# TUI-NICR/EMSANet

Hardware: AMD Instinct MI355X
Metric: images/sec (640x480 RGB-D, bs=32/GPU) fwd+bwd (higher is better)
Workload: dtype f32; 1 GPU; BASELINE.json configs[1]: full EMSANet RGB-D (resnet34-NBt1D x2, SE-add fusion, PPM, semantic+instance+orientation+scene heads), 640x480, bs=32/GPU, f32, train mode (BN batch stats, Dropout2d), step = fwd + bwd (fixed output cotangents) + grad all-reduce + SGD-nesterov update at lr 0 (fixed weights) replayed from a hipGraph; global_batch=32, parallelism=dp1, weights=random init (deterministic), mode=train-hipgraph

## Files before the change

### emsanet_amd/_lib.py

```python
import ctypes
import os
from ctypes import POINTER, Structure, c_char_p, c_float, c_int, c_int8, c_int32, c_int64, c_uint32, c_void_p

LIB_PATH = os.environ.get('EMSA_LIB') or os.path.join(
    os.path.dirname(os.path.abspath(__file__)), 'lib', 'libemsanet_hip.so')


class EmsaPackJob(Structure):
    _fields_ = [('src', c_void_p), ('dst0', c_void_p), ('dst1', c_void_p), ('cout', c_int32),
                ('cin', c_int32), ('kh', c_int32), ('kw', c_int32), ('kind', c_int32),
                ('first_block', c_int32), ('cout_total', c_int32), ('cout_off', c_int32),
                ('cin_total', c_int32), ('cin_off', c_int32)]


class EmsaDropoutJob(Structure):
    _fields_ = [('offset', c_int64), ('c', c_int32), ('layer_id', c_uint32), ('p', c_float),
                ('pad_', c_int32)]


class EmsaConvGeom(Structure):
    _fields_ = [
        ('n_img', c_int32),
        ('in_h', c_int32), ('in_w', c_int32),
        ('out_h', c_int32), ('out_w', c_int32),
# ... 41 lines not shown
    'emsa_conv_relu_bits_words': (c_int64, [c_int64, c_int32]),
    'emsa_conv1d_wino_bnb': (c_int, [_GP, _P, _P, _P, _P, c_int32, _P, c_int32, _P, _P, _P, _P, _P,
                                     c_int32, _P]),
    'emsa_conv_igemm_bnb_t': (c_int, [c_int32, _GP, _P, _P, _P, _P, c_int32, _P, c_int32, _P, _P, _P, _P,
                                      _P, c_int32, _P]),
    'emsa_bn_bwd_apply_rows_t': (c_int, [c_int32, _P, _P, _P, _P, _P, _P, c_int32, c_int32, c_int64,
                                         c_int32, c_int32, _P, _P, _P, _P]),
    'emsa_conv1d_wino': (c_int, [_GP, _P, _P, _P, _P, _P, _P, _P, _P, c_int32, _P, c_int32, c_int32, _P,
                                 _P, _P]),
    'emsa_memset_async': (c_int, [_P, c_int32, c_int64, _P]),
    'emsa_graph_count_nodes': (c_int, [_P, POINTER(c_int32), POINTER(c_int32), POINTER(c_int32)]),
    'emsa_graph_replace_memsets': (c_int, [_P, POINTER(c_int32)]),
    'emsa_dropout2d_mask_batch': (c_int, [_P, _P, c_int32, c_int32, c_int32, c_uint32, _P, _P]),
    'emsa_to_nhwc_t': (c_int, [c_int32, _P, _P, c_int32, c_int32, c_int32, c_int32, c_int64, c_int64,
                               c_int64, c_int64, _P]),
    'emsa_conv1d_wino_resmask_supported': (c_int, [_GP, c_int32]),
    'emsa_conv1d_wino_resmask': (c_int, [_GP, _P, _P, _P, _P, c_int32, _P, _P]),
    'emsa_bn_act_fwd_wbits': (c_int, [_P, _P, _P, _P, _P, _P, c_int32, c_int64, c_int32, c_int32, _P, _P]),
    'emsa_bn_act_fwd_raff': (c_int, [_P] * 8 + [c_int32, c_int64, c_int32, c_int32, _P, c_int32, _P]),
    'emsa_bn_bwd_reduce_wbits': (c_int, [_P, _P, _P, _P, _P, _P, c_int32, c_int64, c_int32, _P, _P]),
    'emsa_bn_bwd_apply_wbits': (c_int, [_P] * 8 + [c_int32, c_int32, c_int64, c_int32, c_int32] + [_P] * 5),
    'emsa_conv1d_wino_inbn': (c_int, [_GP, _P, _P, _P, _P, _P, _P, _P, c_int32, _P, _P]),
    'emsa_conv_wgrad_inbn': (c_int, [_GP, _P, _P, _P, _P, _P, _P, _P, _P]),
    'emsa_conv_wgrad_inbn_t': (c_int, [c_int32, _GP, _P, _P, _P, _P, _P, _P, _P, _P]),
    'emsa_conv_wgrad_multi_inbn_t': (c_int, [c_int32, c_int32, _GP, POINTER(c_void_p), POINTER(c_void_p),
                                             POINTER(c_void_p), POINTER(c_void_p), _P,
                                             POINTER(c_void_p), POINTER(c_void_p), _P]),
    'emsa_conv1d_rs_inbn_t': (c_int, [c_int32, _GP, _P, _P, _P, _P, _P, _P, _P, c_int32, _P]),
    'emsa_bn_bwd_reduce_aff_t': (c_int, [c_int32, _P, _P, _P, _P, _P, _P, c_int32, c_int64, c_int32, _P, _P]),
    'emsa_bn_bwd_apply_aff_t': (c_int, [c_int32, _P, _P, _P, _P, _P, _P, _P, _P, c_int32, c_int32, c_int64,
# ... 247 lines not shown
```

### emsanet_amd/csrc/conv_mfma.hip

```cpp
#include "common.h"

#include <type_traits>
#include <vector>

#include "prof.h"

namespace {

struct ProfSlotImpl {
  hipEvent_t a, b;
  int cls;
  double flops, bytes;
};
std::vector<ProfSlotImpl> g_prof_pool;
size_t g_prof_used = 0;
int g_prof_every = 0;
int g_prof_seen[kProfClasses] = {0};
double g_prof_next_flops = 0.0;
const char* const kProfNames[kProfClasses] = {
    "conv_igemm_kernel<128,128,2,2>", "conv_igemm_kernel<128,64,4,2>",
    "conv_igemm_kernel<64,64,2,2>",   "conv_igemm_kernel<128,32,4,1>",
    "conv_wgrad_kernel<64,32,7,2,1,2>", "conv_wgrad_kernel<128,128,1,2,2,1> (unused)",
    "conv_wgrad_kernel<64,64,1,2,2,1>", "conv_wgrad_kernel<64,64,3,2,2,1>|conv_wgrad1d_wino_kernel<64,64> (1-D convs)",
    "conv1d_wino_kernel (1-D 3x1/1x3 convs)", "conv_h_kernel (16-bit igemm)",
// ... 956 lines not shown
  const bool dok = co0 + col4 < p.n_ch, xok = ci0 + col4 < p.k_ch;
  const uint32_t dadd = dok ? (uint32_t)(co0 + col4) * ES : 0u, dmask = dok ? 0u : kOOB;
  const uint32_t xadd = xok ? (uint32_t)(ci0 + col4) * ES : 0u, xmask = xok ? 0u : kOOB;

  typename Raw4<T>::type re_raw[2], rx_raw[4];
  float4 bsum = emsa_zero4();
  uint32_t x_real = 0;
  float* const xbnS = smem + NP * 4 * (BCO + BCI);
  if constexpr (XBN) {
    if (tid < 2 * BCI) {
      const int ch = ci0 + (tid & (BCI - 1));
      const float* src = tid < BCI ? p.in_scale : p.in_shift;
      xbnS[tid] = ch < p.k_ch ? src[ch] : 0.f;
    }
  }
  auto load_regs = [&](int s) {
    const int k = s * PK + lane - 1;
    const bool valid = lane < XROWS && k >= 0 && k < p.M;
    const uint32_t ku = valid ? (uint32_t)k : 0u;
    const uint32_t img = fast_div(ku, p.div_al);
    const uint32_t line = fast_div(ku, p.div_l);
    const int b_ = (int)(ku - __umul24(line, (uint32_t)p.L));
    const int a_ = (int)(line - __umul24(img, (uint32_t)p.A));
    const int a2 = a_ + dline;
    const bool in_line = valid && b_ < p.Lr;
    const uint32_t off_d = in_line
        ? (__umul24(img, (uint32_t)p.dy_simg) + __umul24((uint32_t)a_, (uint32_t)p.dy_sa) +
           __umul24((uint32_t)b_, (uint32_t)p.dy_sb)) * ES : kOOB;
    const uint32_t off_x = (in_line && a2 >= 0 && a2 < p.A)
        ? (__umul24(img, (uint32_t)p.in_simg) + __umul24((uint32_t)a2, (uint32_t)p.in_sa) +
           __umul24((uint32_t)b_, (uint32_t)p.in_sb)) * ES : kOOB;
    const uint32_t off_xl = b_ == p.L - 1 ? kOOB : off_x;
    const uint32_t off_xr = b_ == 0 ? kOOB : off_x;
    const int l0 = (2 * pr) * 4;
    const uint32_t o_e0 = (uint32_t)__builtin_amdgcn_ds_bpermute(l0 + 4, (int)off_d);
    const uint32_t o_e1 = (uint32_t)__builtin_amdgcn_ds_bpermute(l0 + 8, (int)off_d);
    const uint32_t o_d0 = (uint32_t)__builtin_amdgcn_ds_bpermute(l0, (int)off_xl);
    const uint32_t o_d1 = (uint32_t)__builtin_amdgcn_ds_bpermute(l0 + 4, (int)off_x);
    const uint32_t o_d2 = (uint32_t)__builtin_amdgcn_ds_bpermute(l0 + 8, (int)off_x);
    const uint32_t o_d3 = (uint32_t)__builtin_amdgcn_ds_bpermute(l0 + 12, (int)off_xr);
    re_raw[0] = buf_ld4raw<T>(rs_dy, (o_e0 + dadd) | dmask);
    re_raw[1] = buf_ld4raw<T>(rs_dy, (o_e1 + dadd) | dmask);
    rx_raw[0] = buf_ld4raw<T>(rs_in, (o_d0 + xadd) | xmask);
    rx_raw[1] = buf_ld4raw<T>(rs_in, (o_d1 + xadd) | xmask);
    rx_raw[2] = buf_ld4raw<T>(rs_in, (o_d2 + xadd) | xmask);
    rx_raw[3] = buf_ld4raw<T>(rs_in, (o_d3 + xadd) | xmask);
    if constexpr (XBN)
      x_real = (~o_d0 >> 31) | ((~o_d1 >> 31) << 1) | ((~o_d2 >> 31) << 2) | ((~o_d3 >> 31) << 3);
  };
  auto add4 = [](const float4& a, const float4& b) {
    return make_float4(a.x + b.x, a.y + b.y, a.z + b.z, a.w + b.w);
  };
  auto sub4 = [](const float4& a, const float4& b) {
    return make_float4(a.x - b.x, a.y - b.y, a.z - b.z, a.w - b.w);
  };
  auto store_lds = [&]() {
    const float4 re[2] = {raw_f4(re_raw[0], (T*)nullptr), raw_f4(re_raw[1], (T*)nullptr)};
    float4 rx[4] = {raw_f4(rx_raw[0], (T*)nullptr), raw_f4(rx_raw[1], (T*)nullptr),
                    raw_f4(rx_raw[2], (T*)nullptr), raw_f4(rx_raw[3], (T*)nullptr)};
    if constexpr (XBN) {
      typedef float f2 __attribute__((ext_vector_type(2)));
// ... 1489 lines not shown
```

### emsanet_amd/csrc/conv_wino.hip

```cpp
#include <cstdlib>

#include "common.h"
#include "prof.h"

namespace {

constexpr int kWK = 16;
constexpr int kWLD = kWK;
constexpr int kPairs = 32;

typedef unsigned int u32x4w __attribute__((ext_vector_type(4)));
typedef __bf16 wbf16x8 __attribute__((ext_vector_type(8)));
constexpr uint32_t kOOBw = 0x80000000u;
__device__ __forceinline__ __amdgpu_buffer_rsrc_t wrsrc(const void* p, uint32_t bytes) {
  return __builtin_amdgcn_make_buffer_rsrc(const_cast<void*>(p), 0, (int)bytes, 0x00020000);
}
__device__ __forceinline__ float4 wbuf_ld4(__amdgpu_buffer_rsrc_t r, uint32_t off) {
  return __builtin_bit_cast(float4, __builtin_amdgcn_raw_buffer_load_b128(r, (int)off, 0, 0));
}
__device__ __forceinline__ float4 wbuf_ld4s(__amdgpu_buffer_rsrc_t r, uint32_t voff, uint32_t soff) {
  return __builtin_bit_cast(float4,
                            __builtin_amdgcn_raw_buffer_load_b128(r, (int)voff, (int)soff, 0));
}
typedef float wf32x2 __attribute__((ext_vector_type(2)));
// ... 31 lines not shown

__device__ __forceinline__ int wswz(int row, int c4) {
  return row * kWLD + (c4 ^ (((row >> 2) & 3) << 2));
}

__device__ __forceinline__ uint32_t wdiv(uint32_t n, uint32_t mul, uint32_t sh) {
  return (__umulhi(n, mul) + n) >> sh;
}

#ifndef EMSA_WINO_ST_AUX
#define EMSA_WINO_ST_AUX 0
#endif
#ifndef EMSA_WINO_PRIO
#define EMSA_WINO_PRIO 2
#endif
template <int kWN, bool BF16 = false, bool BNB = false, bool INBN = false>
__global__ __launch_bounds__(256, kWN == 64 ? (BNB ? 4 : 5) : 6) void conv1d_wino_kernel(const WinoArgs p) {
  constexpr int NT = kWN / 32;
  constexpr int NC4 = kWN / 4;
  constexpr int RG = 256 / NC4;
  constexpr int PXI = 64 / RG;
  constexpr int BLD = 4 * kWN * 4 / 256;
  extern __shared__ __attribute__((aligned(16))) float smem[];
  float* const As = smem;
  float* const Bs = smem + 4 * kPairs * kWLD;
  float* const Ts = Bs + 4 * kWN * kWLD;

  const int tid = threadIdx.x, lane = tid & 63, wave = __builtin_amdgcn_readfirstlane(tid >> 6);
  const int l31 = lane & 31, lh = lane >> 5;
  const int wg = emsa_xcd_remap(blockIdx.x, gridDim.x);
  const int nt = wg % p.tiles_n, mt = wg / p.tiles_n;
  const int q0 = mt * kPairs, n0 = nt * kWN;
// ... 13 lines not shown
      int al = 0;
      if (q < p.MP) {
        const int line = (int)wdiv((uint32_t)q, p.mul_pl, p.sh_pl);
        const int pp = q - line * p.PL;
        const int img = (int)wdiv((uint32_t)line, p.mul_a, p.sh_a);
        const int a = line - img * p.A;
        const int b = 2 * pp - 1 + rr;
        if (b >= 0 && b < p.L)
          off = (uint32_t)(img * p.in_simg + a * p.in_sa + b * p.in_sb + c4) * 4u;
        al = a;
      }
      a_base[j] = off;
      a_line[j] = al;
    }
  };
  setup_a(mt);
#pragma unroll
  for (int j = 0; j < BLD; ++j) {
    const int rowid = (tid >> 2) + 64 * j;
    const int comp = rowid / kWN, n = n0 + (rowid % kWN);
    b_voff[j] = n < p.n_ch ? (uint32_t)((comp * p.n_ch + n) * p.k_ch + c4) * 4u : kOOBw;
  }
  auto set_row = [&](int r) {
    const int dr = p.R == 3 ? r - 1 : 0;
#pragma unroll
    for (int j = 0; j < 2; ++j) {
      const int al = a_line[j] + dr;
      const bool ok = !(a_base[j] & kOOBw) && al >= 0 && al < p.A;
      a_voff[j] = ok ? a_base[j] + (uint32_t)(dr * p.in_sa * 4) : kOOBw;
    }
  };
  const uint32_t last_oob = (p.ksteps_c - 1) * kWK + c4 < p.c_in ? 0u : kOOBw;
  float4 ra[2], rb[BLD];
  auto load_regs = [&](int s) {
    const int r = s >= 2 * p.ksteps_c ? 2 : (s >= p.ksteps_c ? 1 : 0);
    const int ch = (s - r * p.ksteps_c) * kWK;
    if (ch == 0) set_row(r);
    const uint32_t sa = (uint32_t)ch * 4u, sb = (uint32_t)(r * p.c_in + ch) * 4u;
    const uint32_t pm = ch + kWK > p.c_in ? 0xFFFFFFFFu : 0u;
#pragma unroll
    for (int j = 0; j < 2; ++j) ra[j] = wbuf_ld4s(rs_in, a_voff[j] | (last_oob & pm), sa);
#pragma unroll
    for (int j = 0; j < BLD; ++j) rb[j] = wbuf_ld4s(rs_u, b_voff[j] | (last_oob & pm), sb);
  };
  auto store_lds = [&](int s) {
    if constexpr (INBN) {
      const int kt = p.ksteps_c * kWK;
      const float4 sc = emsa_ld4(Ts + s * kWK + c4), sh = emsa_ld4(Ts + kt + s * kWK + c4);
#pragma unroll
// ... 9 lines not shown
                            __builtin_amdgcn_fmed3f(hi.y, 0.f, cap));
      }
    }
#pragma unroll
    for (int j = 0; j < 2; ++j) emsa_st4(As + wswz((tid >> 2) + 64 * j, c4), ra[j]);
#pragma unroll
    for (int j = 0; j < BLD; ++j) emsa_st4(Bs + wswz((tid >> 2) + 64 * j, c4), rb[j]);
  };

  const int ra_ = wave == 0 ? 0 : wave == 2 ? 2 : 1;
  const int rb_ = wave == 2 ? 1 : wave == 3 ? 3 : 2;
  const float sg = wave == 1 ? 1.f : -1.f;

  load_regs(0);
  f32x16 acc[NT];
#pragma unroll
  for (int t = 0; t < NT; ++t)
#pragma unroll
    for (int r = 0; r < 16; ++r) acc[t][r] = 0.f;

  if constexpr (INBN) {
    const int kt = p.ksteps_c * kWK;
    for (int i = tid; i < kt; i += 256) {
      Ts[i] = i < p.c_in ? p.in_scale[i] : 0.f;
      Ts[kt + i] = i < p.c_in ? p.in_shift[i] : 0.f;
    }
    __syncthreads();
  }
  store_lds(0);
  __syncthreads();
  for (int s = 0; s < p.ksteps; ++s) {
    const bool has_next = s + 1 < p.ksteps;
#if EMSA_WINO_PRIO == 2
    __builtin_amdgcn_s_setprio(3);
#endif
    if (has_next) load_regs(s + 1);
    const int sw = ((l31 >> 2) & 3) << 2;
    const float* a0 = As + (ra_ * kPairs + l31) * kWLD;
    const float* a1 = As + (rb_ * kPairs + l31) * kWLD;
    const float* b = Bs + (wave * kWN + l31) * kWLD;
#if EMSA_WINO_PRIO != 0
    __builtin_amdgcn_s_setprio(1);
#endif
    if constexpr (BF16) {
      const int c0 = (lh << 2) ^ sw, c1 = ((lh + 2) << 2) ^ sw;
      const float4 p0 = emsa_ld4(a0 + c0), q0 = emsa_ld4(a1 + c0);
// ... 12 lines not shown
        acc[u] = __builtin_amdgcn_mfma_f32_32x32x16_bf16(va, vb, acc[u], 0, 0, 0);
      }
    } else {
#pragma unroll
    for (int t = 0; t < kWK / 8; ++t) {
      const int co = ((lh + 2 * t) << 2) ^ sw;
      const float4 x0 = emsa_ld4(a0 + co), x1 = emsa_ld4(a1 + co);
      const wf32x2 sg2 = {sg, sg};
      const wf32x2 vlo = __builtin_elementwise_fma(wf32x2{x1.x, x1.y}, sg2, wf32x2{x0.x, x0.y});
      const wf32x2 vhi = __builtin_elementwise_fma(wf32x2{x1.z, x1.w}, sg2, wf32x2{x0.z, x0.w});
      const float4 v = make_float4(vlo.x, vlo.y, vhi.x, vhi.y);
      float4 fb[NT];
#pragma unroll
      for (int u = 0; u < NT; ++u) fb[u] = emsa_ld4(b + u * 32 * kWLD + co);
#pragma unroll
      for (int u = 0; u < NT; ++u)
        acc[u] = __builtin_amdgcn_mfma_f32_32x32x2f32(v.x, fb[u].x, acc[u], 0, 0, 0);
#pragma unroll
      for (int u = 0; u < NT; ++u)
        acc[u] = __builtin_amdgcn_mfma_f32_32x32x2f32(v.y, fb[u].y, acc[u], 0, 0, 0);
#pragma unroll
      for (int u = 0; u < NT; ++u)
        acc[u] = __builtin_amdgcn_mfma_f32_32x32x2f32(v.z, fb[u].z, acc[u], 0, 0, 0);
#pragma unroll
      for (int u = 0; u < NT; ++u)
        acc[u] = __builtin_amdgcn_mfma_f32_32x32x2f32(v.w, fb[u].w, acc[u], 0, 0, 0);
    }
    }
#if EMSA_WINO_PRIO != 0
    __builtin_amdgcn_s_setprio(0);
#endif
    __syncthreads();
    if (has_next) store_lds(s + 1);
    __syncthreads();
  }

  constexpr int SLD = kWN + 4;
  constexpr int HP = kPairs / 2;
  constexpr uint32_t kNoPix = 0xFFFFFFFFu;
  float* const stage = smem;
  const int col4 = tid % NC4, n = n0 + col4 * 4;
  const int rgi = tid / NC4;
  const bool nok = n < p.n_ch;
  uint32_t lane_pix = kNoPix;
  {
    const int q = q0 + (lane >> 1);
    if (q < p.MP) {
      const int line = (int)wdiv((uint32_t)q, p.mul_pl, p.sh_pl);
      const int pp = q - line * p.PL;
      const int img = (int)wdiv((uint32_t)line, p.mul_a, p.sh_a);
      const int a = line - img * p.A;
      const int b = 2 * pp + (lane & 1);
      if (b < p.L) lane_pix = (uint32_t)(img * p.px_simg + a * p.px_sa + b * p.px_sb);
    }
  }
  wf32x2 ylo[PXI], yhi[PXI];
  uint32_t opix[PXI];
  bool ok[PXI];
  const float4 bv = (nok && p.bias) ? emsa_ld4(p.bias + n) : emsa_zero4();
  const wf32x2 blo = {bv.x, bv.y}, bhi = {bv.z, bv.w};
  const float sgo = (rgi & 1) ? -1.f : 1.f;
  const wf32x2 sg2o = {sgo, sgo};
  const int m03row = (rgi & 1) ? 3 : 0;
#pragma unroll
  for (int k = 0; k < PXI; ++k) {
    const uint32_t o = (uint32_t)__builtin_amdgcn_ds_bpermute((rgi + RG * k) * 4, (int)lane_pix);
    ok[k] = nok && o != kNoPix;
    opix[k] = o;
  }
  const __amdgpu_buffer_rsrc_t rs_out = wrsrc(p.out, kOOBw);
  const __amdgpu_buffer_rsrc_t rs_res = wrsrc(p.residual, kOOBw);
  const __amdgpu_buffer_rsrc_t rs_msk = wrsrc(p.mask_src, kOOBw);
  const __amdgpu_buffer_rsrc_t rs_mb = wrsrc(p.mask_bits, kOOBw);
  float4 rres[PXI], rmsk[PXI];
  wu32x2 rbits[PXI];
#pragma unroll
  for (int k = 0; k < PXI; ++k) {
    const bool live = ok[k];
    if (p.residual)
      rres[k] = wbuf_ld4(rs_res, live ? (opix[k] * (uint32_t)p.ld_res + (uint32_t)n) * 4u : kOOBw);
    if (p.mask_src)
      rmsk[k] = wbuf_ld4(rs_msk, live ? (opix[k] * (uint32_t)p.ld_mask + (uint32_t)n) * 4u : kOOBw);
    if constexpr (kWN == 64) {
      if (p.mask_bits)
        rbits[k] = __builtin_bit_cast(
            wu32x2, __builtin_amdgcn_raw_buffer_load_b64(
                        rs_mb, (int)(live ? (opix[k] * (uint32_t)p.tiles_n + (uint32_t)nt) * 8u
                                          : kOOBw), 0, 0));
    }
  }
#pragma unroll
  for (int h = 0; h < 2; ++h) {
  if (h) __syncthreads();
#pragma unroll
  for (int t = 0; t < NT; ++t)
#pragma unroll
    for (int r = 8 * h; r < 8 * h + 8; ++r) {
      const int row = (r & 3) + 8 * (r >> 2) + 4 * lh;
      stage[(wave * HP + row - HP * h) * SLD + t * 32 + l31] = acc[t][r];
    }
  __syncthreads();
#pragma unroll
  for (int k = h * (PXI / 2); k < (h + 1) * (PXI / 2); ++k) {
    const int px = rgi + RG * k;
    const int prl = (px >> 1) - HP * h;
    const float4 m1 = emsa_ld4(stage + (1 * HP + prl) * SLD + col4 * 4);
    const float4 m2 = emsa_ld4(stage + (2 * HP + prl) * SLD + col4 * 4);
    const float4 m03 = emsa_ld4(stage + (m03row * HP + prl) * SLD + col4 * 4);
    const wf32x2 tlo = wf32x2{m2.x, m2.y} + wf32x2{m03.x, m03.y};
    const wf32x2 thi = wf32x2{m2.z, m2.w} + wf32x2{m03.z, m03.w};
    ylo[k] = __builtin_elementwise_fma(tlo, sg2o, wf32x2{m1.x, m1.y}) + blo;
    yhi[k] = __builtin_elementwise_fma(thi, sg2o, wf32x2{m1.z, m1.w}) + bhi;
  }
  }

  if (p.stats != nullptr) {
    __syncthreads();
    float* red = smem;
    float* tmean = smem + RG * kWN;
    int* scnt = reinterpret_cast<int*>(tmean + kWN);
    wf32x2 s1lo = {0.f, 0.f}, s1hi = {0.f, 0.f};
    float wgt[PXI];
    int cnt = 0;
#pragma unroll
    for (int k = 0; k < PXI; ++k) {
      wgt[k] = ok[k] ? 1.f : 0.f;
      const wf32x2 w2 = {wgt[k], wgt[k]};
      s1lo = __builtin_elementwise_fma(ylo[k], w2, s1lo);
      s1hi = __builtin_elementwise_fma(yhi[k], w2, s1hi);
      cnt += ok[k] ? 1 : 0;
    }
// ... 26 lines not shown
    }
    __syncthreads();
    emsa_st4(red + rgi * kWN + col4 * 4, make_float4(s2lo.x, s2lo.y, s2hi.x, s2hi.y));
    __syncthreads();
    if (tid < kWN && n0 + tid < p.n_ch) {
      float a2 = 0.f;
#pragma unroll
      for (int g = 0; g < RG; ++g) a2 += red[g * kWN + tid];
      p.stats[((size_t)1 * p.tiles_m + mt) * p.n_ch + n0 + tid] = a2;
    }
  }

  {
    wf32x2 sclo = {1.f, 1.f}, schi = {1.f, 1.f}, shlo = {0.f, 0.f}, shhi = {0.f, 0.f};
    constexpr bool bnb = BNB;
    const bool affine = p.scale != nullptr && !bnb;
    if (p.scale != nullptr && nok) {
      const float4 sc = emsa_ld4(p.scale + n), sh = emsa_ld4(p.shift + n);
      sclo = wf32x2{sc.x, sc.y}; schi = wf32x2{sc.z, sc.w};
      shlo = wf32x2{sh.x, sh.y}; shhi = wf32x2{sh.z, sh.w};
    }
    wf32x2 mulo = {0.f, 0.f}, muhi = {0.f, 0.f};
    wf32x2 b0lo = {0.f, 0.f}, b0hi = {0.f, 0.f}, b1lo = {0.f, 0.f}, b1hi = {0.f, 0.f};
    if (bnb && nok) {
      const float4 mu = emsa_ld4(p.bnb_mean + n);
      mulo = wf32x2{mu.x, mu.y}; muhi = wf32x2{mu.z, mu.w};
    }
#pragma unroll
    for (int k = 0; k < PXI; ++k) {
      const bool live = ok[k];
      wf32x2 vlo = ylo[k], vhi = yhi[k];
      if (affine) {
        vlo = __builtin_elementwise_fma(vlo, sclo, shlo);
        vhi = __builtin_elementwise_fma(vhi, schi, shhi);
      }
      auto gate = [&](float4& q) {
        const uint32_t t0 = rbits[k].x >> col4, t1 = rbits[k].y >> col4;
        q.x = __uint_as_float(__float_as_uint(q.x) & (uint32_t)__builtin_amdgcn_sbfe((int)t0, 0, 1));
        q.y = __uint_as_float(__float_as_uint(q.y) & (uint32_t)__builtin_amdgcn_sbfe((int)t0, 16, 1));
        q.z = __uint_as_float(__float_as_uint(q.z) & (uint32_t)__builtin_amdgcn_sbfe((int)t1, 0, 1));
        q.w = __uint_as_float(__float_as_uint(q.w) & (uint32_t)__builtin_amdgcn_sbfe((int)t1, 16, 1));
      };
      if (p.residual) {
        float4 rr = rres[k];
        if constexpr (kWN == 64) {
          if (p.mask_res) gate(rr);
        }
        vlo += wf32x2{rr.x, rr.y};
        vhi += wf32x2{rr.z, rr.w};
      }
      float4 v = make_float4(vlo.x, vlo.y, vhi.x, vhi.y);
      if constexpr (bnb) {
        const float4 tt = rmsk[k];
        const wf32x2 alo = __builtin_elementwise_fma(wf32x2{tt.x, tt.y}, sclo, shlo);
        const wf32x2 ahi = __builtin_elementwise_fma(wf32x2{tt.z, tt.w}, schi, shhi);
        const float lv = live ? 1.f : 0.f;
        v.x = alo.x > 0.f ? v.x * lv : 0.f; v.y = alo.y > 0.f ? v.y * lv : 0.f;
        v.z = ahi.x > 0.f ? v.z * lv : 0.f; v.w = ahi.y > 0.f ? v.w * lv : 0.f;
        const wf32x2 glo = {v.x, v.y}, ghi = {v.z, v.w};
        b0lo += glo; b0hi += ghi;
        b1lo = __builtin_elementwise_fma(glo, wf32x2{tt.x, tt.y} - mulo, b1lo);
        b1hi = __builtin_elementwise_fma(ghi, wf32x2{tt.z, tt.w} - muhi, b1hi);
      } else if (p.mask_src) {
        const float4 mm = rmsk[k];
        v.x = mm.x > 0.f ? v.x : 0.f; v.y = mm.y > 0.f ? v.y : 0.f;
        v.z = mm.z > 0.f ? v.z : 0.f; v.w = mm.w > 0.f ? v.w : 0.f;
      }
      if constexpr (kWN == 64) {
        if (p.mask_bits && !p.mask_res) gate(v);
      }
      if (p.act == EMSA_ACT_RELU) {
        v.x = fmaxf(v.x, 0.f); v.y = fmaxf(v.y, 0.f);
        v.z = fmaxf(v.z, 0.f); v.w = fmaxf(v.w, 0.f);
      }
      {
        const uint32_t off = live ? (opix[k] * (uint32_t)p.ld_out + (uint32_t)n) * 4u : kOOBw;
        __builtin_amdgcn_raw_buffer_store_b128(__builtin_bit_cast(u32x4w, v), rs_out, (int)off, 0,
                                               EMSA_WINO_ST_AUX);
      }
      if constexpr (kWN == 64) {
        if (p.relu_bits) {
          const uint64_t b0 = __ballot(live && v.x > 0.f), b1 = __ballot(live && v.y > 0.f);
          const uint64_t b2 = __ballot(live && v.z > 0.f), b3 = __ballot(live && v.w > 0.f);
          const int sh16 = (lane >> 4) * 16;
          if (col4 == 0 && opix[k] != kNoPix)
            p.relu_bits[(size_t)opix[k] * p.tiles_n + nt] =
                ((b0 >> sh16) & 0xFFFFull) | (((b1 >> sh16) & 0xFFFFull) << 16) |
                (((b2 >> sh16) & 0xFFFFull) << 32) | (((b3 >> sh16) & 0xFFFFull) << 48);
        }
      }
    }
    if constexpr (bnb) {
      __syncthreads();
      float* red0 = smem;
      float* red1 = smem + RG * kWN;
      emsa_st4(red0 + rgi * kWN + col4 * 4, make_float4(b0lo.x, b0lo.y, b0hi.x, b0hi.y));
// ... 254 lines not shown

extern "C" int emsa_conv1d_wino_stats_rows(const EmsaConvGeom* g) {
  if (!emsa_conv1d_wino_supported(g)) return EMSA_E_SHAPE;
  const bool aw = g->kw == 3;
  const int L = aw ? g->out_w : g->out_h, A = aw ? g->out_h : g->out_w;
  const long mp = (long)g->n_img * A * ((L + 1) / 2);
  return (int)((mp + kPairs - 1) / kPairs);
}

static int wino_wn() {
  static const int forced_wn = [] {
    const char* e = getenv("EMSA_WINO_WN");
    return e ? atoi(e) : 0;
  }();
  return forced_wn == 32 || forced_wn == 64 ? forced_wn : 64;
}

static int conv1d_wino_impl(const EmsaConvGeom* g, const float* in, const float* u, float* out,
                            const float* bias, float* stats, const float* scale,
                            const float* shift, const float* residual, int32_t ld_res,
                            const float* mask_src, int32_t ld_mask, int32_t act,
                            const uint64_t* mask_bits, uint64_t* relu_bits,
                            const float* bnb_mean, const float* bnb_invstd, float* bnb_out,
                            int32_t bnb_rows_alloc, const float* in_scale, const float* in_shift,
                            void* stream, bool mask_res = false) {
  if (!emsa_conv1d_wino_supported(g)) return EMSA_E_SHAPE;
  if ((in_scale == nullptr) != (in_shift == nullptr)) return EMSA_E_ARG;
  if (!in || !u || !out) return EMSA_E_ARG;
  if ((scale == nullptr) != (shift == nullptr)) return EMSA_E_ARG;
  auto al16 = [](const void* q) { return (((uintptr_t)q) & 15) == 0; };
// ... 48 lines not shown
  a.u_bytes = (uint32_t)((size_t)4 * g->n_ch * a.k_ch * sizeof(float));
  magic((uint32_t)a.PL, a.mul_pl, a.sh_pl);
  magic((uint32_t)a.A, a.mul_a, a.sh_a);
  if (in_scale && (a.R != 1 || bnb_out || wn != 64)) return EMSA_E_SHAPE;
  const size_t lds_main = (size_t)(4 * kPairs + 4 * wn) * kWLD * sizeof(float) +
                          (in_scale ? (size_t)2 * a.ksteps_c * kWK * sizeof(float) : 0);
  const size_t lds_epi = (size_t)4 * (kPairs / 2) * (wn + 4) * sizeof(float);
  const size_t lds = lds_main > lds_epi ? lds_main : lds_epi;
  const double flops = 2.0 * g->n_img * H * W * (double)g->k_ch * g->n_ch * 3.0 * a.R;
  const int ps = emsa_prof_begin(a.R == 3 ? kProfClassWino3x3 : kProfClassWino, flops,
                                 (hipStream_t)stream);
  static const bool bf16 = [] {
    const char* e = getenv("EMSA_BF16_MFMA");
    return e && e[0] == '1';
  }();
  if (in_scale) {
    hipLaunchKernelGGL((conv1d_wino_kernel<64, false, false, true>),
                       dim3(a.tiles_m * a.tiles_n), dim3(256), lds, (hipStream_t)stream, a);
  } else if (bnb_out) {
    if (wn != 64) return EMSA_E_SHAPE;
    hipLaunchKernelGGL((conv1d_wino_kernel<64, false, true>), dim3(a.tiles_m * a.tiles_n),
                       dim3(256), lds, (hipStream_t)stream, a);
  } else if (wn == 64 && bf16)
    hipLaunchKernelGGL((conv1d_wino_kernel<64, true>), dim3(a.tiles_m * a.tiles_n), dim3(256), lds,
                       (hipStream_t)stream, a);
  else if (wn == 64)
    hipLaunchKernelGGL((conv1d_wino_kernel<64, false>), dim3(a.tiles_m * a.tiles_n), dim3(256),
                       lds, (hipStream_t)stream, a);
  else
    hipLaunchKernelGGL((conv1d_wino_kernel<32, false>), dim3(a.tiles_m * a.tiles_n), dim3(256),
                       lds, (hipStream_t)stream, a);
// ... 53 lines not shown
```

### include/emsanet_hip.h

```cpp
#ifndef EMSANET_HIP_H
#define EMSANET_HIP_H

#include <stdint.h>

#ifdef __cplusplus
extern "C" {
#endif

#define EMSA_OK 0
#define EMSA_E_SHAPE (-1)
#define EMSA_E_ARG (-2)
#define EMSA_E_LAUNCH (-3)

#define EMSA_ACT_NONE 0
#define EMSA_ACT_RELU 1

#define EMSA_DT_F32 0
#define EMSA_DT_BF16 1
#define EMSA_DT_F16 2

const char* emsa_arch(void);
int emsa_version(void);
int emsa_set_batch_invariant(int on);

// ... 22 lines not shown
int emsa_conv_wgrad(const EmsaConvGeom* g, const float* in, const float* dout, float* dw,
                    float* dbias, float* ws, void* stream);

int emsa_conv1d_wino_supported(const EmsaConvGeom* g);
int emsa_conv1d_wino_stats_rows(const EmsaConvGeom* g);
int64_t emsa_conv_relu_bits_words(int64_t pixels, int32_t n_ch);
int emsa_conv1d_wino(const EmsaConvGeom* g, const float* in, const float* u, float* out,
                     const float* bias, float* stats, const float* scale, const float* shift,
                     const float* residual, int32_t ld_res, const float* mask_src,
                     int32_t ld_mask, int32_t act, const uint64_t* mask_bits,
                     uint64_t* relu_bits, void* stream);
int emsa_conv1d_wino_bnb(const EmsaConvGeom* g, const float* dy, const float* u, float* out,
                         const float* residual, int32_t ld_res, const float* t, int32_t ld_t,
                         const float* bn_scale, const float* bn_shift, const float* bn_mean,
                         const float* bn_invstd, float* partial, int32_t rows_alloc, void* stream);
int emsa_conv1d_wino_resmask_supported(const EmsaConvGeom* g, int32_t ld_res);
int emsa_conv1d_wino_resmask(const EmsaConvGeom* g, const float* dy, const float* u, float* out,
                             const float* residual, int32_t ld_res, const uint64_t* res_bits,
                             void* stream);
int emsa_conv1d_wino_inbn(const EmsaConvGeom* g, const float* in, const float* u, float* out,
                          const float* bias, float* stats, const float* in_scale,
                          const float* in_shift, int32_t act, uint64_t* relu_bits, void* stream);
int emsa_conv_wgrad_inbn(const EmsaConvGeom* g, const float* in, const float* dout, float* dw,
                         float* dbias, float* ws, const float* in_scale, const float* in_shift,
                         void* stream);
int emsa_pack_wino(const float* w_oihw, float* u, float* u_dgrad, int32_t cout, int32_t cin,
                   int32_t rows, void* stream);
int emsa_pack_wino_packed(const float* w_packed, float* u, int32_t n_ch, int32_t k_ch,
                          int32_t rows, int32_t flip, void* stream);
int emsa_conv_wino2d_supported(const EmsaConvGeom* g);
// ... 584 lines not shown
```

Baseline: 348.0 images/s.

## Specialise 1-D Winograd conv epilogues at compile time and lean wgrad address math

Adds compile-time-specialised variants of the 1-D Winograd conv kernel, keyed on a bitmask of epilogue options (bias, relu, relu bits, stats, masks, residual) and dispatched through a switch on the host. Each variant drops runtime branches, simplifies A-operand addressing for R==1, and zeroes the accumulator through the first MFMA instead of an explicit clear. Separately, the fp32 wgrad kernel swaps per-lane divisions for a wave-uniform base plus carry corrections, and builds out-of-bounds offsets with a saturating add. The risks are more template instantiations (larger binary and compile time) and new edge-case correctness paths in the indexing. An env var and API toggle can switch the specialisation off.

```diff
diff --git a/emsanet_amd/_lib.py b/emsanet_amd/_lib.py
--- a/emsanet_amd/_lib.py
+++ b/emsanet_amd/_lib.py
@@ -79,6 +79,8 @@
     'emsa_dropout2d_mask_batch': (c_int, [_P, _P, c_int32, c_int32, c_int32, c_uint32, _P, _P]),
     'emsa_to_nhwc_t': (c_int, [c_int32, _P, _P, c_int32, c_int32, c_int32, c_int32, c_int64, c_int64,
                                c_int64, c_int64, _P]),
+    'emsa_conv1d_wino_set_spec': (c_int, [c_int32]),
+    'emsa_conv1d_wino_spec_launches': (c_int, []),
     'emsa_conv1d_wino_resmask_supported': (c_int, [_GP, c_int32]),
     'emsa_conv1d_wino_resmask': (c_int, [_GP, _P, _P, _P, _P, c_int32, _P, _P]),
     'emsa_bn_act_fwd_wbits': (c_int, [_P, _P, _P, _P, _P, _P, c_int32, c_int64, c_int32, c_int32, _P, _P]),
diff --git a/emsanet_amd/csrc/conv_mfma.hip b/emsanet_amd/csrc/conv_mfma.hip
--- a/emsanet_amd/csrc/conv_mfma.hip
+++ b/emsanet_amd/csrc/conv_mfma.hip
@@ -994,22 +994,58 @@
       xbnS[tid] = ch < p.k_ch ? src[ch] : 0.f;
     }
   }
+  constexpr bool LEAN = !BF16 && sizeof(T) == 4;
+  int ln_dr = 0, ln_da = 0;
+  uint32_t ln_cd = 0, ln_cx = 0;
+  if constexpr (LEAN) {
+    const uint32_t d = lane < XROWS ? (uint32_t)(XROWS - 1 - lane) : 0u;
+    const uint32_t dI = fast_div(d, p.div_al), dLn = fast_div(d, p.div_l);
+    ln_dr = (int)(d - dLn * (uint32_t)p.L);
+    ln_da = (int)(dLn - dI * (uint32_t)p.A);
+    ln_cd = (dI * (uint32_t)p.dy_simg + (uint32_t)ln_da * (uint32_t)p.dy_sa +
+             (uint32_t)ln_dr * (uint32_t)p.dy_sb) * ES;
+    ln_cx = (dI * (uint32_t)p.in_simg + (uint32_t)ln_da * (uint32_t)p.in_sa +
+             (uint32_t)ln_dr * (uint32_t)p.in_sb) * ES;
+  }
   auto load_regs = [&](int s) {
     const int k = s * PK + lane - 1;
     const bool valid = lane < XROWS && k >= 0 && k < p.M;
+    int b_, a2;
+    bool in_line;
+    uint32_t off_d, off_x;
+    if constexpr (LEAN) {
+      const uint32_t K1 = (uint32_t)__builtin_amdgcn_readfirstlane(s * PK + PK);
+      const uint32_t I1 = fast_div(K1, p.div_al), Ln1 = fast_div(K1, p.div_l);
+      const int b1 = (int)(K1 - Ln1 * (uint32_t)p.L), a1 = (int)(Ln1 - I1 * (uint32_t)p.A);
+      const uint32_t base_d = (I1 * (uint32_t)p.dy_simg + (uint32_t)a1 * (uint32_t)p.dy_sa +
+                               (uint32_t)b1 * (uint32_t)p.dy_sb) * ES;
+      const uint32_t base_x = (I1 * (uint32_t)p.in_simg + (uint32_t)(a1 + dline) * (uint32_t)p.in_sa +
+                               (uint32_t)b1 * (uint32_t)p.in_sb) * ES;
+      const uint32_t cb_d = (uint32_t)(p.L * p.dy_sb - p.dy_sa) * ES, ca_d = (uint32_t)(p.A * p.dy_sa - p.dy_simg) * ES;
+      const uint32_t cb_x = (uint32_t)(p.L * p.in_sb - p.in_sa) * ES, ca_x = (uint32_t)(p.A * p.in_sa - p.in_simg) * ES;
+      const int br = b1 - ln_dr, bm = br >> 31;
+      b_ = br + (bm & p.L);
+      const int ar = a1 - ln_da + bm, am = ar >> 31;
+      a2 = ar + (am & p.A) + dline;
+      in_line = valid && b_ < p.Lr;
+      off_d = in_line ? base_d - ln_cd + ((uint32_t)bm & cb_d) + ((uint32_t)am & ca_d) : kOOB;
+      off_x = (in_line && a2 >= 0 && a2 < p.A)
+                  ? base_x - ln_cx + ((uint32_t)bm & cb_x) + ((uint32_t)am & ca_x) : kOOB;
+    } else {
     const uint32_t ku = valid ? (uint32_t)k : 0u;
     const uint32_t img = fast_div(ku, p.div_al);
     const uint32_t line = fast_div(ku, p.div_l);
-    const int b_ = (int)(ku - __umul24(line, (uint32_t)p.L));
+    b_ = (int)(ku - __umul24(line, (uint32_t)p.L));
     const int a_ = (int)(line - __umul24(img, (uint32_t)p.A));
-    const int a2 = a_ + dline;
-    const bool in_line = valid && b_ < p.Lr;
-    const uint32_t off_d = in_line
+    a2 = a_ + dline;
+    in_line = valid && b_ < p.Lr;
+    off_d = in_line
         ? (__umul24(img, (uint32_t)p.dy_simg) + __umul24((uint32_t)a_, (uint32_t)p.dy_sa) +
            __umul24((uint32_t)b_, (uint32_t)p.dy_sb)) * ES : kOOB;
-    const uint32_t off_x = (in_line && a2 >= 0 && a2 < p.A)
+    off_x = (in_line && a2 >= 0 && a2 < p.A)
         ? (__umul24(img, (uint32_t)p.in_simg) + __umul24((uint32_t)a2, (uint32_t)p.in_sa) +
            __umul24((uint32_t)b_, (uint32_t)p.in_sb)) * ES : kOOB;
+    }
     const uint32_t off_xl = b_ == p.L - 1 ? kOOB : off_x;
     const uint32_t off_xr = b_ == 0 ? kOOB : off_x;
     const int l0 = (2 * pr) * 4;
@@ -1019,12 +1055,22 @@
     const uint32_t o_d1 = (uint32_t)__builtin_amdgcn_ds_bpermute(l0 + 4, (int)off_x);
     const uint32_t o_d2 = (uint32_t)__builtin_amdgcn_ds_bpermute(l0 + 8, (int)off_x);
     const uint32_t o_d3 = (uint32_t)__builtin_amdgcn_ds_bpermute(l0 + 12, (int)off_xr);
+    if constexpr (LEAN) {
+      const uint32_t dsat = dok ? dadd : 0xFFFFFFFFu, xsat = xok ? xadd : 0xFFFFFFFFu;
+      re_raw[0] = buf_ld4raw<T>(rs_dy, __builtin_elementwise_add_sat(o_e0, dsat));
+      re_raw[1] = buf_ld4raw<T>(rs_dy, __builtin_elementwise_add_sat(o_e1, dsat));
+      rx_raw[0] = buf_ld4raw<T>(rs_in, __builtin_elementwise_add_sat(o_d0, xsat));
+      rx_raw[1] = buf_ld4raw<T>(rs_in, __builtin_elementwise_add_sat(o_d1, xsat));
+      rx_raw[2] = buf_ld4raw<T>(rs_in, __builtin_elementwise_add_sat(o_d2, xsat));
+      rx_raw[3] = buf_ld4raw<T>(rs_in, __builtin_elementwise_add_sat(o_d3, xsat));
+    } else {
     re_raw[0] = buf_ld4raw<T>(rs_dy, (o_e0 + dadd) | dmask);
     re_raw[1] = buf_ld4raw<T>(rs_dy, (o_e1 + dadd) | dmask);
     rx_raw[0] = buf_ld4raw<T>(rs_in, (o_d0 + xadd) | xmask);
     rx_raw[1] = buf_ld4raw<T>(rs_in, (o_d1 + xadd) | xmask);
     rx_raw[2] = buf_ld4raw<T>(rs_in, (o_d2 + xadd) | xmask);
     rx_raw[3] = buf_ld4raw<T>(rs_in, (o_d3 + xadd) | xmask);
+    }
     if constexpr (XBN)
       x_real = (~o_d0 >> 31) | ((~o_d1 >> 31) << 1) | ((~o_d2 >> 31) << 2) | ((~o_d3 >> 31) << 3);
   };
diff --git a/emsanet_amd/csrc/conv_wino.hip b/emsanet_amd/csrc/conv_wino.hip
--- a/emsanet_amd/csrc/conv_wino.hip
+++ b/emsanet_amd/csrc/conv_wino.hip
@@ -1,4 +1,6 @@
+#include <atomic>
 #include <cstdlib>
+#include <type_traits>
 
 #include "common.h"
 #include "prof.h"
@@ -69,8 +71,22 @@
 #ifndef EMSA_WINO_PRIO
 #define EMSA_WINO_PRIO 2
 #endif
-template <int kWN, bool BF16 = false, bool BNB = false, bool INBN = false>
+enum : int {
+  kOBias = 1, kORelu = 2, kORBits = 4, kOStats = 8, kOMBits = 16, kORes = 32, kOMRes = 64
+};
+template <int kWN, bool BF16 = false, bool BNB = false, bool INBN = false, int OPT = -1>
 __global__ __launch_bounds__(256, kWN == 64 ? (BNB ? 4 : 5) : 6) void conv1d_wino_kernel(const WinoArgs p) {
+  constexpr bool SPEC = OPT >= 0;
+  static_assert(!SPEC || (kWN == 64 && !BF16), "specialised epilogues: fp32, 64-channel tiles");
+  const bool f_bias = SPEC ? (OPT & kOBias) != 0 : p.bias != nullptr;
+  const bool f_relu = SPEC ? (OPT & kORelu) != 0 : p.act == EMSA_ACT_RELU;
+  const bool f_rbits = SPEC ? (OPT & kORBits) != 0 : p.relu_bits != nullptr;
+  const bool f_stats = SPEC ? (OPT & kOStats) != 0 : p.stats != nullptr;
+  const bool f_mbits = SPEC ? (OPT & kOMBits) != 0 : p.mask_bits != nullptr;
+  const bool f_res = SPEC ? (OPT & kORes) != 0 : p.residual != nullptr;
+  const bool f_mres = SPEC ? (OPT & kOMRes) != 0 : p.mask_res != 0;
+  const bool f_scale = SPEC ? BNB : p.scale != nullptr;
+  const bool f_msrc = SPEC ? BNB : p.mask_src != nullptr;
   constexpr int NT = kWN / 32;
   constexpr int NC4 = kWN / 4;
   constexpr int RG = 256 / NC4;
@@ -114,7 +130,24 @@
       a_line[j] = al;
     }
   };
-  setup_a(mt);
+  if constexpr (SPEC) {
+    const int rr0 = tid >> 7, q = q0 + ((tid >> 2) & 31);
+    a_voff[0] = a_voff[1] = kOOBw;
+    if (q < p.MP) {
+      const int line = (int)wdiv((uint32_t)q, p.mul_pl, p.sh_pl);
+      const int pp = q - line * p.PL;
+      const int img = (int)wdiv((uint32_t)line, p.mul_a, p.sh_a);
+      const int a = line - img * p.A;
+      const int base = img * p.in_simg + a * p.in_sa + c4;
+#pragma unroll
+      for (int j = 0; j < 2; ++j) {
+        const int b = 2 * pp - 1 + rr0 + 2 * j;
+        if (b >= 0 && b < p.L) a_voff[j] = (uint32_t)(base + b * p.in_sb) * 4u;
+      }
+    }
+  } else {
+    setup_a(mt);
+  }
 #pragma unroll
   for (int j = 0; j < BLD; ++j) {
     const int rowid = (tid >> 2) + 64 * j;
@@ -122,7 +155,7 @@
     b_voff[j] = n < p.n_ch ? (uint32_t)((comp * p.n_ch + n) * p.k_ch + c4) * 4u : kOOBw;
   }
   auto set_row = [&](int r) {
-    const int dr = p.R == 3 ? r - 1 : 0;
+    const int dr = !SPEC && p.R == 3 ? r - 1 : 0;
 #pragma unroll
     for (int j = 0; j < 2; ++j) {
       const int al = a_line[j] + dr;
@@ -133,6 +166,14 @@
   const uint32_t last_oob = (p.ksteps_c - 1) * kWK + c4 < p.c_in ? 0u : kOOBw;
   float4 ra[2], rb[BLD];
   auto load_regs = [&](int s) {
+    if constexpr (SPEC) {
+      const uint32_t so = (uint32_t)(s * kWK) * 4u;
+#pragma unroll
+      for (int j = 0; j < 2; ++j) ra[j] = wbuf_ld4s(rs_in, a_voff[j], so);
+#pragma unroll
+      for (int j = 0; j < BLD; ++j) rb[j] = wbuf_ld4s(rs_u, b_voff[j], so);
+      return;
+    }
     const int r = s >= 2 * p.ksteps_c ? 2 : (s >= p.ksteps_c ? 1 : 0);
     const int ch = (s - r * p.ksteps_c) * kWK;
     if (ch == 0) set_row(r);
@@ -172,10 +213,12 @@
 
   load_regs(0);
   f32x16 acc[NT];
-#pragma unroll
-  for (int t = 0; t < NT; ++t)
-#pragma unroll
-    for (int r = 0; r < 16; ++r) acc[t][r] = 0.f;
+  if constexpr (!SPEC) {
+#pragma unroll
+    for (int t = 0; t < NT; ++t)
+#pragma unroll
+      for (int r = 0; r < 16; ++r) acc[t][r] = 0.f;
+  }
 
   if constexpr (INBN) {
     const int kt = p.ksteps_c * kWK;
@@ -187,7 +230,8 @@
   }
   store_lds(0);
   __syncthreads();
-  for (int s = 0; s < p.ksteps; ++s) {
+  auto kstep = [&](int s, auto first_c) {
+    constexpr bool first = decltype(first_c)::value;
     const bool has_next = s + 1 < p.ksteps;
 #if EMSA_WINO_PRIO == 2
     __builtin_amdgcn_s_setprio(3);
@@ -230,8 +274,15 @@
 #pragma unroll
       for (int u = 0; u < NT; ++u) fb[u] = emsa_ld4(b + u * 32 * kWLD + co);
 #pragma unroll
-      for (int u = 0; u < NT; ++u)
-        acc[u] = __builtin_amdgcn_mfma_f32_32x32x2f32(v.x, fb[u].x, acc[u], 0, 0, 0);
+      for (int u = 0; u < NT; ++u) {
+        if (first && t == 0) {
+          const f32x16 zero = {0.f, 0.f, 0.f, 0.f, 0.f, 0.f, 0.f, 0.f,
+                               0.f, 0.f, 0.f, 0.f, 0.f, 0.f, 0.f, 0.f};
+          acc[u] = __builtin_amdgcn_mfma_f32_32x32x2f32(v.x, fb[u].x, zero, 0, 0, 0);
+        } else {
+          acc[u] = __builtin_amdgcn_mfma_f32_32x32x2f32(v.x, fb[u].x, acc[u], 0, 0, 0);
+        }
+      }
 #pragma unroll
       for (int u = 0; u < NT; ++u)
         acc[u] = __builtin_amdgcn_mfma_f32_32x32x2f32(v.y, fb[u].y, acc[u], 0, 0, 0);
@@ -249,6 +300,12 @@
     __syncthreads();
     if (has_next) store_lds(s + 1);
     __syncthreads();
+  };
+  if constexpr (SPEC) {
+    kstep(0, std::true_type{});
+    for (int s = 1; s < p.ksteps; ++s) kstep(s, std::false_type{});
+  } else {
+    for (int s = 0; s < p.ksteps; ++s) kstep(s, std::false_type{});
   }
 
   constexpr int SLD = kWN + 4;
@@ -273,7 +330,7 @@
   wf32x2 ylo[PXI], yhi[PXI];
   uint32_t opix[PXI];
   bool ok[PXI];
-  const float4 bv = (nok && p.bias) ? emsa_ld4(p.bias + n) : emsa_zero4();
+  const float4 bv = (nok && f_bias) ? emsa_ld4(p.bias + n) : emsa_zero4();
   const wf32x2 blo = {bv.x, bv.y}, bhi = {bv.z, bv.w};
   const float sgo = (rgi & 1) ? -1.f : 1.f;
   const wf32x2 sg2o = {sgo, sgo};
@@ -293,12 +350,12 @@
 #pragma unroll
   for (int k = 0; k < PXI; ++k) {
     const bool live = ok[k];
-    if (p.residual)
+    if (f_res)
       rres[k] = wbuf_ld4(rs_res, live ? (opix[k] * (uint32_t)p.ld_res + (uint32_t)n) * 4u : kOOBw);
-    if (p.mask_src)
+    if (f_msrc)
       rmsk[k] = wbuf_ld4(rs_msk, live ? (opix[k] * (uint32_t)p.ld_mask + (uint32_t)n) * 4u : kOOBw);
     if constexpr (kWN == 64) {
-      if (p.mask_bits)
+      if (f_mbits)
         rbits[k] = __builtin_bit_cast(
             wu32x2, __builtin_amdgcn_raw_buffer_load_b64(
                         rs_mb, (int)(live ? (opix[k] * (uint32_t)p.tiles_n + (uint32_t)nt) * 8u
@@ -325,12 +382,16 @@
     const float4 m03 = emsa_ld4(stage + (m03row * HP + prl) * SLD + col4 * 4);
     const wf32x2 tlo = wf32x2{m2.x, m2.y} + wf32x2{m03.x, m03.y};
     const wf32x2 thi = wf32x2{m2.z, m2.w} + wf32x2{m03.z, m03.w};
-    ylo[k] = __builtin_elementwise_fma(tlo, sg2o, wf32x2{m1.x, m1.y}) + blo;
-    yhi[k] = __builtin_elementwise_fma(thi, sg2o, wf32x2{m1.z, m1.w}) + bhi;
-  }
-  }
-
-  if (p.stats != nullptr) {
+    ylo[k] = __builtin_elementwise_fma(tlo, sg2o, wf32x2{m1.x, m1.y});
+    yhi[k] = __builtin_elementwise_fma(thi, sg2o, wf32x2{m1.z, m1.w});
+    if (!SPEC || f_bias) {
+      ylo[k] += blo;
+      yhi[k] += bhi;
+    }
+  }
+  }
+
+  if (f_stats) {
     __syncthreads();
     float* red = smem;
     float* tmean = smem + RG * kWN;
@@ -387,8 +448,8 @@
   {
     wf32x2 sclo = {1.f, 1.f}, schi = {1.f, 1.f}, shlo = {0.f, 0.f}, shhi = {0.f, 0.f};
     constexpr bool bnb = BNB;
-    const bool affine = p.scale != nullptr && !bnb;
-    if (p.scale != nullptr && nok) {
+    const bool affine = f_scale && !bnb;
+    if (f_scale && nok) {
       const float4 sc = emsa_ld4(p.scale + n), sh = emsa_ld4(p.shift + n);
       sclo = wf32x2{sc.x, sc.y}; schi = wf32x2{sc.z, sc.w};
       shlo = wf32x2{sh.x, sh.y}; shhi = wf32x2{sh.z, sh.w};
@@ -414,10 +475,10 @@
         q.z = __uint_as_float(__float_as_uint(q.z) & (uint32_t)__builtin_amdgcn_sbfe((int)t1, 0, 1));
         q.w = __uint_as_float(__float_as_uint(q.w) & (uint32_t)__builtin_amdgcn_sbfe((int)t1, 16, 1));
       };
-      if (p.residual) {
+      if (f_res) {
         float4 rr = rres[k];
         if constexpr (kWN == 64) {
-          if (p.mask_res) gate(rr);
+          if (f_mres) gate(rr);
         }
         vlo += wf32x2{rr.x, rr.y};
         vhi += wf32x2{rr.z, rr.w};
@@ -434,15 +495,21 @@
         b0lo += glo; b0hi += ghi;
         b1lo = __builtin_elementwise_fma(glo, wf32x2{tt.x, tt.y} - mulo, b1lo);
         b1hi = __builtin_elementwise_fma(ghi, wf32x2{tt.z, tt.w} - muhi, b1hi);
-      } else if (p.mask_src) {
+      } else if (f_msrc) {
         const float4 mm = rmsk[k];
         v.x = mm.x > 0.f ? v.x : 0.f; v.y = mm.y > 0.f ? v.y : 0.f;
         v.z = mm.z > 0.f ? v.z : 0.f; v.w = mm.w > 0.f ? v.w : 0.f;
       }
       if constexpr (kWN == 64) {
-        if (p.mask_bits && !p.mask_res) gate(v);
-      }
-      if (p.act == EMSA_ACT_RELU) {
+        if (f_mbits && !f_mres) gate(v);
+      }
+      if constexpr (SPEC) {
+        if (f_relu) {
+          const float inf = __uint_as_float(0x7F800000u);
+          v.x = __builtin_amdgcn_fmed3f(v.x, 0.f, inf); v.y = __builtin_amdgcn_fmed3f(v.y, 0.f, inf);
+          v.z = __builtin_amdgcn_fmed3f(v.z, 0.f, inf); v.w = __builtin_amdgcn_fmed3f(v.w, 0.f, inf);
+        }
+      } else if (f_relu) {
         v.x = fmaxf(v.x, 0.f); v.y = fmaxf(v.y, 0.f);
         v.z = fmaxf(v.z, 0.f); v.w = fmaxf(v.w, 0.f);
       }
@@ -451,8 +518,23 @@
         __builtin_amdgcn_raw_buffer_store_b128(__builtin_bit_cast(u32x4w, v), rs_out, (int)off, 0,
                                                EMSA_WINO_ST_AUX);
       }
-      if constexpr (kWN == 64) {
-        if (p.relu_bits) {
+      if constexpr (SPEC) {
+        if (f_rbits) {
+          const uint64_t b0 = __builtin_amdgcn_ballot_w64(v.x > 0.f);
+          const uint64_t b1 = __builtin_amdgcn_ballot_w64(v.y > 0.f);
+          const uint64_t b2 = __builtin_amdgcn_ballot_w64(v.z > 0.f);
+          const uint64_t b3 = __builtin_amdgcn_ballot_w64(v.w > 0.f);
+          const int sh16 = (lane >> 4) * 16;
+          const uint32_t t0 = (uint32_t)(b0 >> sh16), t1 = (uint32_t)(b1 >> sh16);
+          const uint32_t t2 = (uint32_t)(b2 >> sh16), t3 = (uint32_t)(b3 >> sh16);
+          const wu32x2 word = {__builtin_amdgcn_perm(t1, t0, 0x05040100u),
+                               __builtin_amdgcn_perm(t3, t2, 0x05040100u)};
+          const uint32_t boff = (col4 == 0 && opix[k] != kNoPix)
+                                    ? (opix[k] * (uint32_t)p.tiles_n + (uint32_t)nt) * 8u : kOOBw;
+          __builtin_amdgcn_raw_buffer_store_b64(word, wrsrc(p.relu_bits, kOOBw), (int)boff, 0, 0);
+        }
+      } else if constexpr (kWN == 64) {
+        if (f_rbits) {
           const uint64_t b0 = __ballot(live && v.x > 0.f), b1 = __ballot(live && v.y > 0.f);
           const uint64_t b2 = __ballot(live && v.z > 0.f), b3 = __ballot(live && v.w > 0.f);
           const int sh16 = (lane >> 4) * 16;
@@ -737,6 +819,33 @@
     return e ? atoi(e) : 0;
   }();
   return forced_wn == 32 || forced_wn == 64 ? forced_wn : 64;
+}
+
+static std::atomic<int> g_wino_spec{[] {
+  const char* e = getenv("EMSA_WINO_SPEC");
+  return e && e[0] == '0' ? 0 : 1;
+}()};
+static std::atomic<int> g_wino_spec_launches{0};
+extern "C" int emsa_conv1d_wino_set_spec(int32_t on) {
+  return g_wino_spec.exchange(on ? 1 : 0, std::memory_order_relaxed);
+}
+extern "C" int emsa_conv1d_wino_spec_launches(void) {
+  return g_wino_spec_launches.load(std::memory_order_relaxed);
+}
+
+constexpr int wino_spec_key(bool bnb, bool inbn, int opt) {
+  return opt | (bnb ? 0x100 : 0) | (inbn ? 0x200 : 0);
+}
+static int wino_spec_opt(const WinoArgs& a, int wn, bool bf16) {
+  if (!g_wino_spec.load(std::memory_order_relaxed) || wn != 64 || bf16 || a.R != 1 || (a.c_in % kWK)) return -1;
+  const bool bnb = a.bnb_out != nullptr;
+  if (!bnb && (a.scale || a.mask_src)) return -1;
+  if (a.act != EMSA_ACT_NONE && a.act != EMSA_ACT_RELU) return -1;
+  const int opt = (a.bias ? kOBias : 0) | (a.act == EMSA_ACT_RELU ? kORelu : 0) |
+                  (a.relu_bits ? kORBits : 0) | (a.stats ? kOStats : 0) |
+                  (a.mask_bits ? kOMBits : 0) | (a.residual ? kORes : 0) |
+                  (a.mask_res ? kOMRes : 0);
+  return wino_spec_key(bnb, a.in_scale != nullptr, opt);
 }
 
 static int conv1d_wino_impl(const EmsaConvGeom* g, const float* in, const float* u, float* out,
@@ -815,7 +924,28 @@
     const char* e = getenv("EMSA_BF16_MFMA");
     return e && e[0] == '1';
   }();
-  if (in_scale) {
+  const dim3 grid(a.tiles_m * a.tiles_n);
+#define EMSA_WINO_SPEC_CASE(BNB_, INBN_, OPT_)                                                     \
+  case wino_spec_key(BNB_, INBN_, OPT_):                                                           \
+    hipLaunchKernelGGL((conv1d_wino_kernel<64, false, BNB_, INBN_, OPT_>), grid, dim3(256), lds,   \
+                       (hipStream_t)stream, a);                                                    \
+    break;
+  bool launched = true;
+  switch (wino_spec_opt(a, wn, bf16)) {
+    EMSA_WINO_SPEC_CASE(false, false, kOBias | kORelu | kORBits)
+    EMSA_WINO_SPEC_CASE(false, true, kOBias | kORelu | kORBits)
+    EMSA_WINO_SPEC_CASE(false, false, kOBias | kOStats)
+    EMSA_WINO_SPEC_CASE(false, false, kOMBits)
+    EMSA_WINO_SPEC_CASE(false, false, kORes | kOMBits | kOMRes)
+    EMSA_WINO_SPEC_CASE(false, false, 0)
+    EMSA_WINO_SPEC_CASE(true, false, 0)
+    EMSA_WINO_SPEC_CASE(true, false, kORes)
+    default: launched = false;
+  }
+#undef EMSA_WINO_SPEC_CASE
+  if (launched) {
+    g_wino_spec_launches.fetch_add(1, std::memory_order_relaxed);
+  } else if (in_scale) {
     hipLaunchKernelGGL((conv1d_wino_kernel<64, false, false, true>),
                        dim3(a.tiles_m * a.tiles_n), dim3(256), lds, (hipStream_t)stream, a);
   } else if (bnb_out) {
diff --git a/include/emsanet_hip.h b/include/emsanet_hip.h
--- a/include/emsanet_hip.h
+++ b/include/emsanet_hip.h
@@ -60,6 +60,8 @@
                          const float* residual, int32_t ld_res, const float* t, int32_t ld_t,
                          const float* bn_scale, const float* bn_shift, const float* bn_mean,
                          const float* bn_invstd, float* partial, int32_t rows_alloc, void* stream);
+int emsa_conv1d_wino_set_spec(int32_t on);
+int emsa_conv1d_wino_spec_launches(void);
 int emsa_conv1d_wino_resmask_supported(const EmsaConvGeom* g, int32_t ld_res);
 int emsa_conv1d_wino_resmask(const EmsaConvGeom* g, const float* dy, const float* u, float* out,
                              const float* residual, int32_t ld_res, const uint64_t* res_bits,
```

New measurement: 354.2 images/s, median of 6. +1.8%, better.
